# hermanjakobsen/robotic-ultrasound-imaging

Measured on AMD Instinct MI355X. Metric: env-steps/sec (whole node) at 4096 envs/GPU, random-action rollout, higher is better.
Workload: dtype f32

## Files before the change

robotic-ultrasound-imaging_amd/csrc/usim_device.h:

```cpp
#pragma once
#include <stdint.h>
#include <hip/hip_vector_types.h>

namespace usim {

constexpr int NJ = 7;
constexpr int OBS_DIM = 19;
constexpr int MAXC = 8;
constexpr int N_TOP = 99;
constexpr int LAT_NA = 9;
constexpr int LAT_NC = 11;
constexpr int LINV_BLK = 8;
constexpr int LINV_NBLK = 13;
constexpr int LOG_WIDTH = 53;
constexpr int WG = 64;

enum Field : int {
    F_Q = 0, F_QD = 7, F_Q0 = 14, F_TS = 21, F_TE = 24, F_U0 = 27, F_VBAR = 28, F_FZBAR = 29, F_FZPREV = 30,
    F_DFZ = 31, F_KST = 32, F_KDMP = 33, F_MU = 34, F_T = 35, F_TOUCH = 36, F_EPISODE = 37, F_EPRET = 38,
    F_STATUS = 39, F_NSCALAR = 40,
    F_LAT = 40,
    F_TOTAL_TOP = 40 + 200
};
__host__ __device__ inline size_t scalar_index(int f, size_t i) { return i * F_NSCALAR + f; }
// ... 36 lines not shown

struct DevModel {
    float m7, c7[3], I7[6];
    float site7[3], hand7[3];
    float pcom7[3], pI7[6];
    float torso[3];
    float grot[9];
    float gquat[4];
    float ghat[4], geps;
    float base[3];
    float ikb[3];
    float invw, wfix, wten;
    float armature[NJ];
    const float* tables;
};

struct DevCfg {
    int mode, horizon, early_term, det_traj, rand_solref, rand_pos, rand_fric, torso_drop;
    int pgs_iters, ik_iters, env_offset, adim;
    uint32_t key0, key1;
    float dt, kp_fixed, damping_ratio, kp_min, kp_max, out_pos, out_ori;
    float stiffness, damping, elem_fric, probe_fric, probe_r, probe_hl;
    float probe_hw, probe_tip;
    float probe_cull2;
    float probe_deep0, probe_inv_band;
    float probe_r2, probe_h, probe_ca, probe_cb, probe_cah;
    float top_off, y_range, drop;
    float probe_fric2, rn_scale;
    int probe_geoms;
    int pair;
    int substeps;
    float dt_ctrl;
    float frictionloss;
};

struct DevIO {
    const float* act;
    float* obs; float* rew; uint8_t* done;
    float* term_obs; int* contacts; float* ep_ret; int* ep_len;
    float* act_out;
    int* status_out;
    float* log;
    const uint8_t* mask;
    const float* reset_params;
    int2* items;
    int* count;
    int bank_row0;
    unsigned long long* dbg;
    int refill;
    int nsub;
    int block;
};

__host__ __device__ inline void advance_rollout_block(DevIO& io, size_t rows, int adim) {
    io.obs += rows * OBS_DIM; io.rew += rows; io.done += rows;
    if (io.term_obs) io.term_obs += rows * OBS_DIM;
    if (io.contacts) io.contacts += rows * (1 + MAXC);
    if (io.ep_ret) io.ep_ret += rows;
    if (io.ep_len) io.ep_len += rows;
    if (io.act_out) io.act_out += rows * adim;
}

enum LaunchFlags : int { LF_AUTO_RESET = 1, LF_RANDOM_ACT = 4 };

enum BankField : int { BQ0 = 0, BTS = 7, BTE = 10, BU0 = 13, BKST = 14, BKDMP = 15, BMU = 16, BFZ = 17, BOBS = 18, BSTATUS = 37, BANK_WORDS = 38 };
constexpr int BANK_DEPTH = 256;
// ... 9 lines not shown
```

robotic-ultrasound-imaging_amd/csrc/usim_kernels.hip:

```cpp
#include <hip/hip_runtime.h>
#include <stdint.h>
#include <type_traits>
#include "usim_device.h"
#include "usim_devmath.h"

namespace usim {


constexpr int GE_X = 0;
constexpr int GE_S = 100;
constexpr int GE_SD = 200;
constexpr int GE_A = 300;
constexpr int GE_U = 300;
constexpr int GE_U_WORDS = 144;
constexpr int CG_WORDS = 8;
constexpr int GE_CG = 400;
constexpr int GE_WS = 464;
constexpr int MAXCAND = 16;
constexpr int GE_STRIDE = 548;
static_assert(GE_WS + MAXC * 8 <= GE_STRIDE && GE_CG + (MAXCAND + 1) * CG_WORDS <= GE_STRIDE && GE_U + GE_U_WORDS <= GE_STRIDE, "per-environment LDS block overflow");
static_assert((LAT_NA + 2) * (LAT_NC + 2) <= GE_U_WORDS && LAT_NA * LAT_NC == N_TOP, "padded lattice grid");

constexpr int SOFT16_LDS_WORDS = TB_WORDS + 16 * GE_STRIDE;

// ... 89 lines not shown
    gx = bx * rn; gy = by * rn;
    const float gxi = gx * ipx;
    g = mk(copysignf(gxi * e, p.x), pxok ? copysignf(gxi * el, p.y) : gx, -gy);
    return d;
}

template <int G>
DI void collide_elem(const float* lds, float* recs, const bool valid, const int e, const int gl, const int gbase, const DevModel& M, const DevCfg& C, const float se, const float dz,
                     const f3 Kx, const f3 Ksx, const f3 Ksy, const f3 Ksz, int& nc) {
    const f3 ax = mk(lds[TB_AXIS + 3 * e], lds[TB_AXIS + 3 * e + 1], lds[TB_AXIS + 3 * e + 2]);
    const f3 tip = mk(M.torso[0] + lds[TB_POS + 3 * e], M.torso[1] + lds[TB_POS + 3 * e + 1], M.torso[2] + lds[TB_POS + 3 * e + 2] + dz) + ax * (se - ELEM_R);
    const f3 rel = tip - Kx;
    const f3 p0 = mk(dot(Ksx, rel), dot(Ksy, rel), dot(Ksz, rel));
    const f3 us = mk(dot(Ksx, ax), dot(Ksy, ax), dot(Ksz, ax)) * (-2.f * ELEM_HL);
    f3 g0, g1, gs;
    (void)probe_sdf(C, p0, g0);
    (void)probe_sdf(C, p0 + us, g1);
    const float s0 = dot(g0, us), s1 = dot(g1, us);
    const float tt = clampf(-s0 * rcp_(fmaxf(s1 - s0, 0.f) + SHAFT_EPS), 0.f, 1.f);
    const float dist = probe_sdf(C, madd(p0, us, tt), gs) - ELEM_R;
    const bool hit = valid && (dist < 0.f);
    const f3 nn = (Ksx * gs.x + Ksy * gs.y + Ksz * gs.z) * -1.f;
    const f3 rr = madd(tip, ax, -2.f * ELEM_HL * tt) + nn * (ELEM_R + 0.5f * dist) - Kx;
    const unsigned long long bal = __ballot(hit);
    const unsigned gm = (unsigned)(bal >> gbase) & ((1u << G) - 1u);
    const int slot = nc + __popc(gm & ((1u << gl) - 1u));
    const int sl = (hit && slot < MAXCAND) ? slot : MAXCAND;
    float4* rec = reinterpret_cast<float4*>(&recs[sl * CG_WORDS]);
    rec[0] = make_float4(nn.x, nn.y, nn.z, rr.x);
    rec[1] = make_float4(rr.y, rr.z, __int_as_float(e), dist);
    nc += __popc(gm);
}

DI bool collide_cull(const float* lds, const int e, const DevModel& M, const DevCfg& C, const float se, const float dz, const f3 Kx, const f3 Ksx, const f3 Ksz) {
    const f3 ax = mk(lds[TB_AXIS + 3 * e], lds[TB_AXIS + 3 * e + 1], lds[TB_AXIS + 3 * e + 2]);
    const f3 mid = mk(M.torso[0] + lds[TB_POS + 3 * e], M.torso[1] + lds[TB_POS + 3 * e + 1], M.torso[2] + lds[TB_POS + 3 * e + 2] + dz) + ax * (se - ELEM_R - ELEM_HL);
    const f3 d = mid - (Kx - Ksz * (C.probe_r + C.probe_h - C.probe_tip));
    const f3 v = d - Ksx * clampf(dot(d, Ksx), -C.probe_hl, C.probe_hl);
    return dot(v, v) < C.probe_cull2;
}
template <int G>
DI void collide_queue(const float* lds, const float* queue, const int nq, float* recs, const int gl, const int gbase, const DevModel& M, const DevCfg& C,
                      const float* s_lds, const float dz, const f3 Kx, const f3 Ksx, const f3 Ksy, const f3 Ksz, int& nc) {
    for (int j0 = 0; __any(j0 < nq); j0 += G) {
        const int j = j0 + gl;
        const bool valid = j < nq;
        const int e = valid ? __float_as_int(queue[j]) : 0;
        collide_elem<G>(lds, recs, valid, e, gl, gbase, M, C, s_lds[e], dz, Kx, Ksx, Ksy, Ksz, nc);
    }
}

#define EBF(off) lds[TB_WORDS + eb * GE_STRIDE + (off)]

template <int G>
DI void contact_overflow(float* lds, const int eb, const int gl, const int gbase, const int nc) {
    if (nc > MAXC) {
        group_sync();
        if constexpr (G == 16) {
            const int m = nc < MAXCAND ? nc : MAXCAND;
            const bool cand = gl < m;
            const float4* rec = reinterpret_cast<const float4*>(&EBF(GE_CG + gl * CG_WORDS));
            const float4 r0 = rec[0], r1 = rec[1];
            const float d = cand ? r1.w : 1.0f;
            int rank = 0;
#define USIM_RANK_STEP(I) { const float di = __int_as_float(__builtin_amdgcn_update_dpp(0, __float_as_int(d), 0x150 + I, 0xf, 0xf, true)); \
                                rank += (di < d || (di == d && I < gl)) ? 1 : 0; }
            USIM_RANK_STEP(0) USIM_RANK_STEP(1) USIM_RANK_STEP(2) USIM_RANK_STEP(3) USIM_RANK_STEP(4) USIM_RANK_STEP(5) USIM_RANK_STEP(6) USIM_RANK_STEP(7)
            USIM_RANK_STEP(8) USIM_RANK_STEP(9) USIM_RANK_STEP(10) USIM_RANK_STEP(11) USIM_RANK_STEP(12) USIM_RANK_STEP(13) USIM_RANK_STEP(14) USIM_RANK_STEP(15)
#undef USIM_RANK_STEP
            const bool keep = cand && rank < MAXC;
// ... 159 lines not shown
```

robotic-ultrasound-imaging_amd/csrc/usim_setup.h:

```cpp
#pragma once
#include <cmath>
#include <cstdint>
#include <cstring>
#include <utility>
#include <vector>

#include "../../include/usim.h"
#include "usim_device.h"
#include "usim_robot.h"

namespace usim {

enum class Mapping : int { FULL, RIGID16, SOFT16_W1, SOFT16_W2, SPLIT16, SPLIT8 };
inline bool resolve_mapping(int torso, int lanes_per_env, int waves_per_simd, int n_envs, Mapping* m) {
    if (waves_per_simd < 0 || waves_per_simd > 2) return false;
    if (torso == USIM_TORSO_NONE) { *m = Mapping::RIGID16; return lanes_per_env == 0 || lanes_per_env == 16; }
    if (lanes_per_env != 0 && lanes_per_env != 16 && lanes_per_env != 32 && lanes_per_env != 64) return false;
    const int lanes = lanes_per_env ? lanes_per_env : (waves_per_simd ? 16 : (n_envs <= 4096 ? 32 : 64));
    const int waves = waves_per_simd ? waves_per_simd : (n_envs <= 4096 ? 1 : 2);
    *m = torso == USIM_TORSO_FULL ? Mapping::FULL : lanes == 32 ? Mapping::SPLIT16 : lanes == 64 ? Mapping::SPLIT8 : (waves == 1 ? Mapping::SOFT16_W1 : Mapping::SOFT16_W2);
    return true;
}
constexpr bool soft_torso(Mapping m) { return m != Mapping::FULL && m != Mapping::RIGID16; }
constexpr bool multi_step(Mapping m) { return m != Mapping::FULL; }
constexpr int launch_steps(int remaining, int kmax, int period_left) {
    const int k = remaining < kmax ? remaining : kmax;
    return k < period_left ? k : period_left;
}
static_assert(launch_steps(1000, 256, 1) == 1, "a period with one step left");
static_assert(launch_steps(1000, 256, BANK_DEPTH) == 256 && launch_steps(1000, 64, BANK_DEPTH) == 64, "a period just refilled");
static_assert(launch_steps(1000, 1, BANK_DEPTH) == 1 && launch_steps(1000, 1, 1) == 1, "kmax = 1: one step per launch");
static_assert(launch_steps(3, 256, 200) == 3 && launch_steps(1, 256, BANK_DEPTH) == 1, "remaining smaller than everything");

// ... 203 lines not shown
    for (int id = 0; id < NSH; ++id) {
        const ShellElement& el = sh[id];
        if (el.b != 3) continue;
        const int e = el.a * 11 + el.c;
        std::memcpy(&tb[TB_SHELL + e], &id, sizeof(int));
        for (int k = 0; k < 3; ++k) { tb[TB_POS + e * 3 + k] = el.pos[k]; tb[TB_AXIS + e * 3 + k] = el.axis[k]; }
        for (int d : {0, 1, 4, 5}) if (el.nbr[d] >= 0) L[(size_t)e * N_TOP + sh[el.nbr[d]].a * 11 + sh[el.nbr[d]].c] = -kWTen;
        L[(size_t)e * N_TOP + e] = lattice_diag(el.nn);
    }
    std::vector<double> Li = invert(L, N_TOP);
    for (int i = 0; i < N_TOP; ++i) for (int j = 0; j < N_TOP; ++j) tb[TB_LINV + (size_t)i * LROW + j] = (float)Li[(size_t)i * N_TOP + j];
    return USIM_OK;
}

inline DevCfg translate_config(const usim_config& cfg) {
    DevCfg C{};
    C.mode = cfg.mode; C.horizon = cfg.horizon; C.early_term = cfg.early_termination; C.det_traj = cfg.deterministic_trajectory;
    C.rand_solref = cfg.torso_solref_randomization; C.rand_pos = cfg.initial_probe_pos_randomization; C.rand_fric = cfg.friction_randomization;
    C.torso_drop = cfg.torso_drop; C.pgs_iters = cfg.pgs_iters; C.ik_iters = cfg.ik_iters; C.env_offset = cfg.env_offset; C.adim = (cfg.mode == USIM_MODE_VARIABLE_Z) ? 7 : 6;
    C.key0 = (uint32_t)cfg.seed; C.key1 = (uint32_t)(cfg.seed >> 32);
    C.substeps = cfg.substeps > 1 ? cfg.substeps : 1;
    C.frictionloss = (float)cfg.joint_frictionloss;
    C.dt_ctrl = (float)cfg.control_dt; C.dt = (float)(cfg.control_dt / C.substeps); C.kp_fixed = (float)cfg.kp_fixed; C.damping_ratio = (float)cfg.damping_ratio; C.kp_min = (float)cfg.kp_min;
    C.kp_max = (float)cfg.kp_max; C.out_pos = (float)cfg.out_max_pos; C.out_ori = (float)cfg.out_max_ori; C.stiffness = (float)cfg.stiffness;
    C.damping = (float)cfg.damping; C.elem_fric = (float)cfg.elem_friction; C.probe_fric = (float)cfg.probe_friction;
    C.probe_geoms = cfg.probe_geoms == 2 ? 2 : 1; C.probe_fric2 = (float)cfg.probe_friction2;
    C.pair = (C.probe_geoms == 2 && cfg.pair_model != 0) ? 1 : 0; C.rn_scale = (C.probe_geoms == 2 && !C.pair) ? 0.5f : 1.0f;
    C.probe_r = (float)cfg.probe_radius; C.probe_hl = (float)cfg.probe_halflen; C.probe_hw = (float)cfg.probe_halfwidth; C.probe_tip = (float)cfg.probe_tip;
    {
        const double cb = (cfg.probe_radius - cfg.probe_radius2) / cfg.probe_height, ca = std::sqrt(1.0 - cb * cb);
        C.probe_r2 = (float)cfg.probe_radius2; C.probe_h = (float)cfg.probe_height; C.probe_ca = (float)ca; C.probe_cb = (float)cb;
        C.probe_cah = C.probe_ca * C.probe_h;
        { const double cr = cfg.probe_radius + cfg.probe_height + cfg.probe_halfwidth + 0.025 + 0.0075 + 1e-4; C.probe_cull2 = (float)(cr * cr); }
        C.probe_deep0 = (float)(cfg.probe_radius * (2.0 / 3.0)); C.probe_inv_band = (float)(1.0 / (cfg.probe_radius * (0.96 - 2.0 / 3.0)));
    }
    {
        const int shape = cfg.torso_shape ? 1 : 0;
        C.top_off = (float)kTopOff[shape]; C.y_range = (float)kYRange[shape]; C.drop = (float)(kTorsoZ[shape] - 0.0525 - 0.8);
        if (cfg.torso_drop == 0) C.drop = 0.f;
        C.torso_drop = cfg.torso_drop == 1 ? 1 : 0;
    }
    return C;
}

}
```

robotic-ultrasound-imaging_amd/csrc/usim_step16.h:

```cpp
#pragma once
#include <type_traits>

namespace usim {

template <int N, class F>
DI void static_for(F&& f) {
    if constexpr (N > 0) { static_for<N - 1>(f); f(std::integral_constant<int, N - 1>{}); }
}

template <int CTRL>
DI float dpp0(float v) { return __int_as_float(__builtin_amdgcn_update_dpp(0, __float_as_int(v), CTRL, 0xf, 0xf, true)); }
template <int G> DI int glane() { return (int)(threadIdx.x & (G - 1)); }
template <int G, int K> DI float rbc(float v) {
    if constexpr (G == 16) return dpp0<0x150 + K>(v);
    else {
        const int iv = __float_as_int(v);
        const int t = __builtin_amdgcn_update_dpp(iv, iv, 0x150 + K, 0xf, 0x3, false);
        return __int_as_float(__builtin_amdgcn_update_dpp(t, iv, 0x150 + 8 + K, 0xf, 0xc, false));
    }
}
template <int G, int D> DI float rshr0(float v) {
    const float t = dpp0<0x110 + D>(v);
    if constexpr (G == 16) return t; else return (glane<G>() < D) ? 0.f : t;
}
// ... 135 lines not shown
    arow = arow > 5 ? 5 : arow;
    const float4 j0 = *reinterpret_cast<const float4*>(&xl[arow * 8]), j1 = *reinterpret_cast<const float4*>(&xl[arow * 8 + 4]);
    Jr[0] = j0.x; Jr[1] = j0.y; Jr[2] = j0.z; Jr[3] = j0.w; Jr[4] = j1.x; Jr[5] = j1.y; Jr[6] = j1.z; Jr[7] = j1.w;
}

template <int G>
DI float solve6_task(float* A, float b, const int gl) {
    static_for<6>([&](auto Kc) {
        constexpr int k = decltype(Kc)::value;
        constexpr int lk = TASK_LANE[k];
        const float g = (A[k] - (gl == lk ? 1.f : 0.f)) * rcp_(rbc<G, lk>(A[k]));
#pragma unroll
        for (int c = k + 1; c < 6; ++c) A[c] = fmaf(-g, rbc<G, lk>(A[c]), A[c]);
        b = fmaf(-g, rbc<G, lk>(b), b);
    });
    return b;
}

constexpr int X16_WORDS = 64;
constexpr int X16_RIGID_STRIDE = 84;

#ifndef USIM_WPR16
#define USIM_WPR16 4
#endif
#ifndef USIM_WPR8
#define USIM_WPR8 4
#endif
template <int G> constexpr int wpr() { return G == 16 ? USIM_WPR16 : USIM_WPR8; }
constexpr int MB_POSE = X16_WORDS;
constexpr int MB_OP = MB_POSE + 12;
constexpr int MB_W = MB_OP + 64;
constexpr int MB_Q = MB_W + 16;
constexpr int MB_GOAL = MB_Q + 100;
constexpr int X2_STRIDE = MB_GOAL + 12;
template <int G> constexpr int x2_base() { return TB_WORDS + (64 * wpr<G>() / G) * GE_STRIDE; }
static_assert(x2_base<16>() % 4 == 0 && x2_base<8>() % 4 == 0 && X2_STRIDE % 4 == 0 && MB_OP % 4 == 0 && MB_W % 4 == 0, "mailbox block: 16-byte accesses");
static_assert((x2_base<8>() + 32 * X2_STRIDE) * 4 <= 160 * 1024, "split kernel with 8-lane groups: LDS of a CU");
template <int G> constexpr int arm_cull_rounds() { return 7; }

#if defined(USIM_TSTAMP) || defined(USIM_TSTAMP_NOWAIT)
#define USIM_BAR() do { __syncthreads(); ++nbar; } while (0)
#else
#define USIM_BAR() __syncthreads()
#endif


constexpr int ARM_LDS_WORDS = A16_LANES * AT_STRIDE;
template <int TORSO, int ROLE, int G> constexpr int arm_lds_base();
template <int NE, class WR = NoWarm>
struct Carry {
    float dqj, qdj, q0j;
    Episode ep;
    float s[NE], sd[NE];
    WR wr;
};

template <int TORSO, int ROLE, int G> constexpr int arm_lds_base() {
    return ROLE != 0 ? x2_base<G>() + (64 * wpr<G>() / G) * X2_STRIDE : (TORSO ? SOFT16_LDS_WORDS : 16 * X16_RIGID_STRIDE);
}
static_assert((arm_lds_base<1, 1, 8>() + ARM_LDS_WORDS) * 4 <= 160 * 1024 && arm_lds_base<1, 1, 8>() % 4 == 0 && arm_lds_base<1, 1, 16>() % 4 == 0 && arm_lds_base<1, 0, 16>() % 4 == 0
              && arm_lds_base<0, 0, 16>() % 4 == 0, "arm table behind the LDS blocks of every 16-lane kernel");

template <int TORSO, int MODE, int ROLE, int NT, int G = 16, bool RES = false, class WR = NoWarm>
DI void step16_one(float* lds, const DevModel& M, const DevCfg& C, float* __restrict__ st, const int n, const int npad, const DevIO& io, const int flags, const long long rstep,
                   const bool first_pass, const int sub, int& nbar, Carry<TORSO ? (N_TOP + G - 1) / G : 1, WR>& cy) {
    constexpr bool WARM = !std::is_same<WR, NoWarm>::value;
    static_assert(!WARM || (TORSO == 1 && ROLE == 0) || (TORSO == 1 && MODE == 0), "warm start: the soft-torso kernels");
    constexpr int WPR = (ROLE != 0) ? wpr<G>() : 4;
    constexpr int EPW = 64 / G, EPB = WPR * EPW;
    static_assert(!RES || MODE == 0, "resident state: step launches only");
    constexpr int X2_BASE = x2_base<G>();
    constexpr unsigned GMASK = (G == 16) ? 0xffffu : 0xffu;
    static_assert(G == 16 || (TORSO == 1 && MODE == 0 && ROLE != 0), "8-lane groups: the split soft-torso step only");
    constexpr int NE = TORSO ? (N_TOP + G - 1) / G : 1;
    static_assert(ROLE == 0 || (TORSO == 1 && MODE == 0), "the split kernel is the soft-torso step");
    const int lane = threadIdx.x & 63, wave = (threadIdx.x >> 6) & (WPR - 1);
    constexpr bool RES_HERE = RES && !(ROLE == 2 && G == 16);
    const bool fresh = !RES_HERE || first_pass;
    const int gl = lane & (G - 1), ge = lane / G;
    const int gbase = lane - gl;
    const int eb = wave * EPW + ge;
    const bool auto_reset = (flags & LF_AUTO_RESET) != 0;
    unsigned long long* const dbg = io.dbg;
    const bool refill = (MODE == 1) && io.refill != 0;
    const int item_cnt = refill ? io.count[0] : 1;
    const int item_first = refill ? (int)blockIdx.x * EPB : 0;
    for (int item0 = item_first; item0 < item_cnt; item0 += refill ? (int)gridDim.x * EPB : 1) {
    int env = blockIdx.x * EPB + eb;
    bool valid = env < n;
    int item_ep = 0;
    if (refill) {
        valid = item0 + eb < item_cnt;
        const int2 it = valid ? io.items[item0 + eb] : make_int2(0, 0);
        env = it.x; item_ep = it.y;
    }
    const bool store = valid && gl == 0;
    const int ei = valid ? env : (refill ? 0 : n - 1);
#define LAT(w) st[(size_t)F_LAT * npad + (size_t)ei * LAT_ENV_WORDS + (w)]
// ... 94 lines not shown
    const bool last_sub = sub == C.substeps - 1;
    const int tphys = (MODE == 0) ? (t - 1) * C.substeps + sub : 0;
    const float dt = C.dt, inv_h = rcp_((float)C.horizon);
#if defined(USIM_TSTAMP) || defined(USIM_TSTAMP_NOWAIT)
#define RSTAMP(k) do { if (dbg && blockIdx.x == 0 && (threadIdx.x & (64 * WPR - 1)) == 0) dbg[(ROLE == 2 ? 30 : 20) + (k)] = __builtin_readcyclecounter(); } while (0)
#else
#define RSTAMP(k) do { } while (0)
#endif
#define XSTAMP(k) RSTAMP(20 + (k))
    if constexpr (ROLE == 2) {
        RSTAMP(0);
        float* const mb = &lds[mbo];
        const int* tb_shell = reinterpret_cast<const int*>(lds + TB_SHELL);
        float dz, vz, az;
        torso_motion(C, tphys, dz, vz, az);
        lattice_rhs<G, NE>(lds, eb, gl, M, az, kst, kdmp, true, s_pre, sd_pre);
        lattice_solve<G>(lds, eb, gl, gbase);
        RSTAMP(1);
        USIM_BAR();
        RSTAMP(2);
        const f3 xs = mk(mb[MB_POSE], mb[MB_POSE + 1], mb[MB_POSE + 2]), sy = mk(mb[MB_POSE + 3], mb[MB_POSE + 4], mb[MB_POSE + 5]),
                 sz = mk(mb[MB_POSE + 6], mb[MB_POSE + 7], mb[MB_POSE + 8]);
        const f3 sxc = cross(sy, sz);
        int nq = __float_as_int(mb[MB_POSE + 10]);
#pragma unroll
        for (int i = arm_cull_rounds<G>(); i < NE; ++i) {
            const int eraw = i * G + gl, e = eraw < N_TOP ? eraw : N_TOP - 1;
            const bool cand = (eraw < N_TOP) && collide_cull(lds, e, M, C, s_pre[i], dz, xs, sxc, sz);
            const unsigned gm = (unsigned)(__ballot(cand) >> gbase) & GMASK;
            mb[MB_Q + (cand ? nq + __popc(gm & ((1u << gl) - 1u)) : 99)] = __int_as_float(e);
            nq += __popc(gm);
        }
        group_sync();
        int nc = 0;
        collide_queue<G>(lds, mb + MB_Q, nq, &EB(GE_CG), gl, gbase, M, C, &EB(GE_S), dz, xs, sxc, sy, sz, nc);
        constexpr bool EARLY = G == 8;
        ContactRows P;
        int nc_early = nc, overflow_early = 0, ncmax_early = 0, cel_early[MAXC];
        if constexpr (EARLY) {
            contact_overflow<G>(lds, eb, gl, gbase, nc_early);
            if (nc_early > MAXC) { overflow_early = 1; nc_early = MAXC; }
            group_sync();
#pragma unroll
            for (int k = MAXC; k >= 1; --k) if (ncmax_early == 0 && __any(nc_early >= k)) ncmax_early = k;
#pragma unroll
            for (int k = 0; k < MAXC; ++k) cel_early[k] = (k < nc_early) ? __float_as_int(EB(GE_CG + k * CG_WORDS + 6)) : 0;
            if (ncmax_early > 0) contact_rows<G>(lds, eb, gl, M, C, nc_early, cel_early, vz, P);
        }
        RSTAMP(3);
        USIM_BAR();
        RSTAMP(4);
        if constexpr (!EARLY) contact_overflow<G>(lds, eb, gl, gbase, nc);
        int overflow = 0;
        if (nc > MAXC) { overflow = 1; nc = MAXC; }
        if constexpr (!EARLY) group_sync();
        XSTAMP(0);
        int ncmax = 0;
        if constexpr (EARLY) { nc = nc_early; overflow = overflow_early; ncmax = ncmax_early; }
        else {
#pragma unroll
            for (int k = MAXC; k >= 1; --k) if (ncmax == 0 && __any(nc >= k)) ncmax = k;
        }
        XSTAMP(1);
        float gf[MAXC], W[6] = {0, 0, 0, 0, 0, 0};
        int cel[MAXC];
#pragma unroll
        for (int k = 0; k < MAXC; ++k) { const int ek = __float_as_int(EB(GE_CG + k * CG_WORDS + 6)); gf[k] = 0.f; cel[k] = EARLY ? cel_early[k] : ((k < nc) ? ek : 0); }
        if (ncmax > 0) {
            float alpha[6], vs[6], Lp[21];
#pragma unroll
            for (int a = 0; a < 6; ++a) {
                alpha[a] = mb[MB_OP + 48 + a]; vs[a] = mb[MB_OP + 54 + a];
#pragma unroll
                for (int b = 0; b <= a; ++b) Lp[PK(a, b)] = mb[MB_OP + a * 8 + b];
            }
            XSTAMP(2);
            contact_solve<G, EARLY, true>(lds, eb, gl, M, C, nc, ncmax, cel, Lp, alpha, vs, mu, vz, P, W, gf, dbg, cy.wr);
            XSTAMP(3);
        } else warm_clear(cy.wr);
        if (gl == 0) {
            *reinterpret_cast<float4*>(&mb[MB_W]) = make_float4(W[0], W[1], W[2], W[3]);
            *reinterpret_cast<float4*>(&mb[MB_W + 4]) = make_float4(W[4], W[5], __int_as_float(nc), __int_as_float(overflow));
#pragma unroll
            for (int k = 0; k < MAXC; ++k) { const int sh = tb_shell[cel[k]]; mb[MB_W + 8 + k] = __int_as_float((k < nc) ? sh : -1); }
        }
        RSTAMP(5);
        USIM_BAR();
        RSTAMP(6);
        {
            float acc_e[NE];
#pragma unroll
            for (int i = 0; i < NE; ++i) { const int e = gl + i * G; acc_e[i] = (e < N_TOP) ? EB(GE_A + e) : 0.f; }
#pragma unroll
            for (int k = 0; k < MAXC; ++k) {
#pragma unroll
                for (int i = 0; i < NE; ++i) {
                    const int e = (gl + i * G < N_TOP) ? gl + i * G : N_TOP - 1;
                    acc_e[i] = fmaf(lds[TB_LINV + e * LROW + cel[k]], gf[k], acc_e[i]);
                }
            }
// ... 96 lines not shown
    fk16<G>(at, qj, X, Y, Z, P);
    const f3 rcm = X * at[AT_LCOM] + Y * at[AT_LCOM + 1] + Z * at[AT_LCOM + 2];
    const f3 cm_ = P + rcm;
    const f3 sx = rbc3<G, 7>(X), sy = rbc3<G, 7>(Y), sz = rbc3<G, 7>(Z), xs = rbc3<G, 7>(P);
    const f3 hand = rbc3<G, NJ - 1>(P + X * M.hand7[0] + Y * M.hand7[1] + Z * M.hand7[2]);
    if constexpr (ROLE == 1) {
        {
            float dz_, vz_, az_;
            torso_motion(C, tphys, dz_, vz_, az_);
            const f3 sxc = cross(sy, sz);
            int nq = 0;
#pragma unroll
            for (int i = 0; i < NE; ++i) {
                const int eraw = i * G + gl, e = eraw < N_TOP ? eraw : N_TOP - 1;
                if (eraw < N_TOP) EB(GE_S + eraw) = s_pre[i];
                if (i >= arm_cull_rounds<G>()) continue;
                const bool cand = (eraw < N_TOP) && collide_cull(lds, e, M, C, s_pre[i], dz_, xs, sxc, sz);
                const unsigned gm = (unsigned)(__ballot(cand) >> gbase) & GMASK;
                xl[MB_Q + (cand ? nq + __popc(gm & ((1u << gl) - 1u)) : 99)] = __int_as_float(e);
                nq += __popc(gm);
            }
            if (gl == 0) xl[MB_POSE + 10] = __int_as_float(nq);
        }
        if (gl == 7) {
            float* mbp = xl + MB_POSE;
            mbp[0] = P.x; mbp[1] = P.y; mbp[2] = P.z; mbp[3] = Y.x; mbp[4] = Y.y; mbp[5] = Y.z; mbp[6] = Z.x; mbp[7] = Z.y; mbp[8] = Z.z;
        }
        if constexpr (ROLE == 1) RSTAMP(1);
        USIM_BAR();
        if constexpr (ROLE == 1) RSTAMP(2);
    }

    float act[7] = {0, 0, 0, 0, 0, 0, 0};
    if constexpr (MODE == 0) {
    if constexpr (ROLE != 2) {
    if (flags & LF_RANDOM_ACT) {
        const uint32_t gid = (uint32_t)(C.env_offset + ei);
        const u4 r = philox(gid, (uint32_t)rstep, (uint32_t)((unsigned long long)rstep >> 32), 1u + (uint32_t)(gl & 1), C.key0, C.key1);
        const float ra = __uint_as_float(r.a), rb = __uint_as_float(r.b), rc = __uint_as_float(r.c), rd = __uint_as_float(r.d);
        uint32_t rr[7];
        rr[0] = __float_as_uint(rbc<G, 0>(ra)); rr[1] = __float_as_uint(rbc<G, 0>(rb)); rr[2] = __float_as_uint(rbc<G, 0>(rc)); rr[3] = __float_as_uint(rbc<G, 0>(rd));
        rr[4] = __float_as_uint(rbc<G, 1>(ra)); rr[5] = __float_as_uint(rbc<G, 1>(rb)); rr[6] = __float_as_uint(rbc<G, 1>(rc));
#pragma unroll
        for (int a = 0; a < 7; ++a) {
            const float u = u01(rr[a]);
            const bool sgn = (C.mode == 1) || (C.mode == 3) || (C.mode == 2 && a == 6);
            act[a] = sgn ? 2.f * u - 1.f : u;
            if (C.mode == 3) act[a] *= WRENCH_MAX;
        }
        if (io.act_out && store) {
#pragma unroll
            for (int a = 0; a < 7; ++a) if (a < C.adim) io.act_out[(size_t)ei * C.adim + a] = act[a];
        }
    } else {
#pragma unroll
        for (int a = 0; a < 7; ++a) if (a < C.adim) act[a] = finite_or_zero(io.act[(size_t)ei * C.adim + a]);
    }
    }
    }
    float bias, Mr[NJ];
    f3 w, al, ao;
    {
        const f3 zq = Z * qdj;
        w = prefix_sum<G>(zq);
        const f3 wp = w - zq;
        const f3 dal = cross(wp, zq);
        al = prefix_sum<G>(dal);
        const f3 alp = al - dal;
        const f3 r = mk(P.x - rshr0<G, 1>(P.x), P.y - rshr0<G, 1>(P.y), P.z - rshr0<G, 1>(P.z));
        f3 da = cross(alp, r) + cross(wp, cross(wp, r));
        da.z += (gl == 0) ? GRAV : 0.f;
        ao = prefix_sum<G>(da);
        const f3 ac = ao + cross(al, rcm) + cross(w, cross(w, rcm));
        const float mass = at[AT_MASS];
        const f3 F = ac * mass;
        const float* I = &at[AT_INERTIA];
        const f3 RI0 = mk(X.x * I[0] + Y.x * I[1] + Z.x * I[2], X.x * I[1] + Y.x * I[3] + Z.x * I[4], X.x * I[2] + Y.x * I[4] + Z.x * I[5]);
        const f3 RI1 = mk(X.y * I[0] + Y.y * I[1] + Z.y * I[2], X.y * I[1] + Y.y * I[3] + Z.y * I[4], X.y * I[2] + Y.y * I[4] + Z.y * I[5]);
        const f3 RI2 = mk(X.z * I[0] + Y.z * I[1] + Z.z * I[2], X.z * I[1] + Y.z * I[3] + Z.z * I[4], X.z * I[2] + Y.z * I[4] + Z.z * I[5]);
        float Iw[6];
        Iw[0] = RI0.x * X.x + RI0.y * Y.x + RI0.z * Z.x; Iw[1] = RI0.x * X.y + RI0.y * Y.y + RI0.z * Z.y; Iw[2] = RI0.x * X.z + RI0.y * Y.z + RI0.z * Z.z;
        Iw[3] = RI1.x * X.y + RI1.y * Y.y + RI1.z * Z.y; Iw[4] = RI1.x * X.z + RI1.y * Y.z + RI1.z * Z.z; Iw[5] = RI2.x * X.z + RI2.y * Y.z + RI2.z * Z.z;
        const f3 Nc = symmul(Iw, al) + cross(w, symmul(Iw, w)) + cross(cm_, F);
        const f3 fa = suffix_sum<G>(F), na = suffix_sum<G>(Nc);
        bias = dot(Z, na - cross(P, fa));
// ... 163 lines not shown
        difference_quat(qe, M.gquat, obs + 15);
        if constexpr (MODE == 0) {
            float pe0 = 90.f * (xw.x - tpw.x), pe1 = 90.f * (xw.y - tpw.y);
            pe0 *= pe0; pe1 *= pe1;
            pos_err_norm = sqrt_(pe0 * pe0 + pe1 * pe1);
            pos_rew = 5.f * exp_(-pos_err_norm);
            const float qc[4] = {qe[3], qe[0], qe[1], qe[2]};
            ori_err = 0.2f * distance_quat_goal(qc, M.ghat, M.geps);
            ori_rew = exp_(-ori_err);
            float ve = 45.f * (vbar - 0.04f); ve *= ve;
            vel_rew = exp_(-ve);
            float fe = 0.7f * (fzbar - 5.f); fe *= fe;
            force_e = 3.f * exp_(-fe);
            float de = 0.01f * dfz; de *= de;
            dforce_e = 2.f * exp_(-de);
        }
    };
    float W[6] = {0, 0, 0, 0, 0, 0};
    int ncon = 0, overflow = 0, con_shell[MAXC];
#pragma unroll
    for (int k = 0; k < MAXC; ++k) con_shell[k] = -1;
    if constexpr (ROLE == 1) {
        if (is_task) {
            const int arow = blk ? 3 + comp : comp;
            float* mbo = xl + MB_OP;
            *reinterpret_cast<float4*>(&mbo[arow * 8]) = make_float4(Li[0], Li[1], Li[2], Li[3]);
            mbo[arow * 8 + 4] = Li[4]; mbo[arow * 8 + 5] = Li[5];
            mbo[48 + arow] = alpha_t; mbo[54 + arow] = v6;
        }
        RSTAMP(3);
        USIM_BAR();
        RSTAMP(4);
        precompute();
        RSTAMP(5);
        USIM_BAR();
        RSTAMP(6);
        const float4 w0 = *reinterpret_cast<const float4*>(&xl[MB_W]), w1 = *reinterpret_cast<const float4*>(&xl[MB_W + 4]);
        W[0] = w0.x; W[1] = w0.y; W[2] = w0.z; W[3] = w0.w; W[4] = w1.x; W[5] = w1.y;
        ncon = __float_as_int(w1.z); overflow = __float_as_int(w1.w);
#pragma unroll
        for (int k = 0; k < MAXC; ++k) con_shell[k] = __float_as_int(xl[MB_W + 8 + k]);
    } else if constexpr (TORSO != 0) {
        const int* tb_shell = reinterpret_cast<const int*>(lds + TB_SHELL);
        float dz, vz, az;
        torso_motion(C, tphys, dz, vz, az);
        lattice_rhs<G, NE>(lds, eb, gl, M, az, kst, kdmp, MODE == 0, s_pre, sd_pre);
        USIM_STAMP(dbg, 5);
        int nc = collide_all<G, NE>(lds, eb, gl, gbase, M, C, MODE == 0, s_pre, dz, xs, sy, sz);
        lattice_solve<G>(lds, eb, gl, gbase);
        contact_overflow<G>(lds, eb, gl, gbase, nc);
        USIM_STAMP(dbg, 7);
        if (nc > MAXC) { overflow = 1; nc = MAXC; }
        ncon = nc;
        group_sync();
        int ncmax = 0;
#pragma unroll
        for (int k = MAXC; k >= 1; --k) if (ncmax == 0 && __any(nc >= k)) ncmax = k;
        float gf[MAXC];
        int cel[MAXC];
#pragma unroll
        for (int k = 0; k < MAXC; ++k) { gf[k] = 0.f; cel[k] = (k < nc) ? __float_as_int(EB(GE_CG + k * CG_WORDS + 6)) : 0; }
        if (ncmax > 0) {
            float alpha[6], vs[6], Lp[21];
            static_for<6>([&](auto Ac) {
                constexpr int a = decltype(Ac)::value;
                alpha[a] = rbc<G, TASK_LANE[a]>(alpha_t); vs[a] = rbc<G, TASK_LANE[a]>(v6);
// ... 205 lines not shown
        }
        if (gl == 0) {
            float4* s4 = reinterpret_cast<float4*>(so);
            if (need) {
                so[F_TS] = ts.x; so[F_TS + 1] = ts.y; so[F_TS + 2] = ts.z;
                s4[6] = make_float4(te.x, te.y, te.z, u0);
            }
            s4[7] = make_float4(vbar, fzbar, fzprev, dfz);
            s4[8] = make_float4(kst, kdmp, mu, __int_as_float(t));
            s4[9] = make_float4(__int_as_float(touched), __int_as_float(episode), epret, __int_as_float(status));
        }
    }
    if (refill) group_sync();
    }
    if (MODE == 1 && refill) work_list_close(io);
    USIM_STAMP(dbg, 16);
    if constexpr (ROLE == 1) RSTAMP(9);
#undef RSTAMP
#undef XSTAMP
#undef LAT
#undef EB
}

template <int TORSO, int MODE, int ROLE, int NT, bool MULTI = false, int G = 16, class WR = NoWarm, bool ACTS = false>
DI void step16_body(float* lds, const DevModel& M, const DevCfg& C, float* __restrict__ st, const int n, const int npad, const DevIO& io0, const int flags, const long long rstep) {
    const int S = (MULTI && MODE == 0 && C.substeps > 1) ? C.substeps : 1;
    const int nsub = (MULTI && MODE == 0) ? (io0.nsub > 1 ? io0.nsub : 1) * S : 1;
    DevIO io = io0;
    int nbar = 0;
    Carry<TORSO ? (N_TOP + G - 1) / G : 1, WR> cy;
    int sub = 0;
    long long cstep = rstep;
    for (int ks = 0; ks < nsub; ++ks) {
        step16_one<TORSO, MODE, ROLE, NT, G, MULTI && MODE == 0, WR>(lds, M, C, st, n, npad, io, flags, cstep, ks == 0, sub, nbar, cy);
        const bool ctrl_done = sub == S - 1;
        if (ctrl_done) { sub = 0; ++cstep; } else ++sub;
        if (ks + 1 < nsub) {
            __threadfence_block();
            if constexpr (ROLE != 0) USIM_BAR();
            if (io0.block && ctrl_done) advance_rollout_block(io, (size_t)n, C.adim);
            if constexpr (ACTS) { if (ctrl_done) io.act += (size_t)n * C.adim; }
        }
    }
#if defined(USIM_TSTAMP) || defined(USIM_TSTAMP_NOWAIT)
    if (ROLE != 0 && io0.dbg && blockIdx.x == 0 && (threadIdx.x & (64 * wpr<G>() - 1)) == 0) io0.dbg[ROLE == 1 ? 46 : 47] = (unsigned long long)nbar;
#endif
}

template <int TORSO, int OCC, int MODE, bool MULTI = false, bool WARM = false>
__global__ __launch_bounds__(256) __attribute__((amdgpu_waves_per_eu(OCC, OCC))) void usim_step16_kernel(const DevModel M, const DevCfg C, float* __restrict__ st, int n, int npad,
                                                                                                          const DevIO io, int flags, long long rstep) {
    extern __shared__ __attribute__((aligned(16))) float lds[];
    step16_body<TORSO, MODE, 0, 256, MULTI, 16, typename std::conditional<WARM, WarmOf<16>::type, NoWarm>::type>(lds, M, C, st, n, npad, io, flags, rstep);
}

template <int TORSO, int OCC, bool WARM = false>
__global__ __launch_bounds__(256) __attribute__((amdgpu_waves_per_eu(OCC, OCC))) void usim_step16_acts_kernel(const DevModel M, const DevCfg C, float* __restrict__ st, int n, int npad,
                                                                                                               const DevIO io, int flags, long long rstep) {
    extern __shared__ __attribute__((aligned(16))) float lds[];
    step16_body<TORSO, 0, 0, 256, true, 16, typename std::conditional<WARM, WarmOf<16>::type, NoWarm>::type, true>(lds, M, C, st, n, npad, io, flags, rstep);
}

template <bool MULTI, int G = 16, bool WARM = false>
__global__ __launch_bounds__(128 * wpr<G>()) __attribute__((amdgpu_waves_per_eu(2, 2))) void usim_step32_kernel(const DevModel* __restrict__ Mp, const DevCfg* __restrict__ Cp, float* __restrict__ st, int n, int npad,
                                                                                                                  const DevIO io, int flags, long long rstep) {
    extern __shared__ __attribute__((aligned(16))) float lds[];
    const DevModel& M = *Mp; const DevCfg& C = *Cp;
// ... 19 lines not shown
```

Baseline: 231.8 million.

## Tighten probe cull to element capsule, draw next random action ahead during precompute

Replaces the probe-axis cull test with a capsule test along each element axis, using a new host-computed radius, so fewer shell elements enter the collision queue. In the resident split kernel the arm wave draws the next step's random action while it waits through the precompute barrier and parks it in a mailbox slot, taking the philox draw off the critical path. It also adds an optional early contact-list path with a readlane max over the 16-lane groups, and sets the 16-lane arm cull rounds to zero by default. The tighter cull changes which candidates are kept, so correctness depends on the new bound being conservative.

```diff
diff --git a/robotic-ultrasound-imaging_amd/csrc/usim_device.h b/robotic-ultrasound-imaging_amd/csrc/usim_device.h
--- a/robotic-ultrasound-imaging_amd/csrc/usim_device.h
+++ b/robotic-ultrasound-imaging_amd/csrc/usim_device.h
@@ -92,6 +92,7 @@
     int substeps;
     float dt_ctrl;
     float frictionloss;
+    float probe_cull2c;
 };
 
 struct DevIO {
diff --git a/robotic-ultrasound-imaging_amd/csrc/usim_kernels.hip b/robotic-ultrasound-imaging_amd/csrc/usim_kernels.hip
--- a/robotic-ultrasound-imaging_amd/csrc/usim_kernels.hip
+++ b/robotic-ultrasound-imaging_amd/csrc/usim_kernels.hip
@@ -145,10 +145,18 @@
     nc += __popc(gm);
 }
 
+#ifndef USIM_CULL_CAPSULE
+#define USIM_CULL_CAPSULE 1
+#endif
+constexpr bool CULL_CAPSULE = USIM_CULL_CAPSULE != 0;
 DI bool collide_cull(const float* lds, const int e, const DevModel& M, const DevCfg& C, const float se, const float dz, const f3 Kx, const f3 Ksx, const f3 Ksz) {
     const f3 ax = mk(lds[TB_AXIS + 3 * e], lds[TB_AXIS + 3 * e + 1], lds[TB_AXIS + 3 * e + 2]);
     const f3 mid = mk(M.torso[0] + lds[TB_POS + 3 * e], M.torso[1] + lds[TB_POS + 3 * e + 1], M.torso[2] + lds[TB_POS + 3 * e + 2] + dz) + ax * (se - ELEM_R - ELEM_HL);
     const f3 d = mid - (Kx - Ksz * (C.probe_r + C.probe_h - C.probe_tip));
+    if constexpr (CULL_CAPSULE) {
+        const f3 v = d - ax * clampf(dot(d, ax), -ELEM_HL, ELEM_HL);
+        return dot(v, v) < C.probe_cull2c;
+    }
     const f3 v = d - Ksx * clampf(dot(d, Ksx), -C.probe_hl, C.probe_hl);
     return dot(v, v) < C.probe_cull2;
 }
diff --git a/robotic-ultrasound-imaging_amd/csrc/usim_setup.h b/robotic-ultrasound-imaging_amd/csrc/usim_setup.h
--- a/robotic-ultrasound-imaging_amd/csrc/usim_setup.h
+++ b/robotic-ultrasound-imaging_amd/csrc/usim_setup.h
@@ -1,4 +1,5 @@
 #pragma once
+#include <algorithm>
 #include <cmath>
 #include <cstdint>
 #include <cstring>
@@ -268,6 +269,11 @@
         C.probe_r2 = (float)cfg.probe_radius2; C.probe_h = (float)cfg.probe_height; C.probe_ca = (float)ca; C.probe_cb = (float)cb;
         C.probe_cah = C.probe_ca * C.probe_h;
         { const double cr = cfg.probe_radius + cfg.probe_height + cfg.probe_halfwidth + 0.025 + 0.0075 + 1e-4; C.probe_cull2 = (float)(cr * cr); }
+        {
+            const double hh = std::hypot(cfg.probe_halflen, cfg.probe_halfwidth);
+            const double rp = std::max(std::hypot(hh, cfg.probe_height) + cfg.probe_radius, hh + cfg.probe_radius2), cr = rp + 0.0075 + 1e-4;
+            C.probe_cull2c = (float)(cr * cr);
+        }
         C.probe_deep0 = (float)(cfg.probe_radius * (2.0 / 3.0)); C.probe_inv_band = (float)(1.0 / (cfg.probe_radius * (0.96 - 2.0 / 3.0)));
     }
     {
diff --git a/robotic-ultrasound-imaging_amd/csrc/usim_step16.h b/robotic-ultrasound-imaging_amd/csrc/usim_step16.h
--- a/robotic-ultrasound-imaging_amd/csrc/usim_step16.h
+++ b/robotic-ultrasound-imaging_amd/csrc/usim_step16.h
@@ -191,11 +191,23 @@
 constexpr int MB_W = MB_OP + 64;
 constexpr int MB_Q = MB_W + 16;
 constexpr int MB_GOAL = MB_Q + 100;
-constexpr int X2_STRIDE = MB_GOAL + 12;
+#ifndef USIM_DRAW_AHEAD
+#define USIM_DRAW_AHEAD 1
+#endif
+constexpr bool DRAW_AHEAD = USIM_DRAW_AHEAD != 0;
+#ifndef USIM_LIST_AHEAD
+#define USIM_LIST_AHEAD 0
+#endif
+constexpr bool LIST_AHEAD = USIM_LIST_AHEAD != 0;
+constexpr int MB_ACT = MB_GOAL + 12;
+constexpr int X2_STRIDE = MB_ACT + (DRAW_AHEAD ? 8 : 0);
 template <int G> constexpr int x2_base() { return TB_WORDS + (64 * wpr<G>() / G) * GE_STRIDE; }
-static_assert(x2_base<16>() % 4 == 0 && x2_base<8>() % 4 == 0 && X2_STRIDE % 4 == 0 && MB_OP % 4 == 0 && MB_W % 4 == 0, "mailbox block: 16-byte accesses");
+static_assert(x2_base<16>() % 4 == 0 && x2_base<8>() % 4 == 0 && X2_STRIDE % 4 == 0 && MB_OP % 4 == 0 && MB_W % 4 == 0 && MB_ACT % 4 == 0, "mailbox block: 16-byte accesses");
 static_assert((x2_base<8>() + 32 * X2_STRIDE) * 4 <= 160 * 1024, "split kernel with 8-lane groups: LDS of a CU");
-template <int G> constexpr int arm_cull_rounds() { return 7; }
+#ifndef USIM_ARM_CULL16
+#define USIM_ARM_CULL16 0
+#endif
+template <int G> constexpr int arm_cull_rounds() { return G == 16 ? USIM_ARM_CULL16 : 7; }
 
 #if defined(USIM_TSTAMP) || defined(USIM_TSTAMP_NOWAIT)
 #define USIM_BAR() do { __syncthreads(); ++nbar; } while (0)
@@ -220,9 +232,10 @@
 static_assert((arm_lds_base<1, 1, 8>() + ARM_LDS_WORDS) * 4 <= 160 * 1024 && arm_lds_base<1, 1, 8>() % 4 == 0 && arm_lds_base<1, 1, 16>() % 4 == 0 && arm_lds_base<1, 0, 16>() % 4 == 0
               && arm_lds_base<0, 0, 16>() % 4 == 0, "arm table behind the LDS blocks of every 16-lane kernel");
 
-template <int TORSO, int MODE, int ROLE, int NT, int G = 16, bool RES = false, class WR = NoWarm>
+template <int TORSO, int MODE, int ROLE, int NT, int G = 16, bool RES = false, class WR = NoWarm, bool AHEAD = false>
 DI void step16_one(float* lds, const DevModel& M, const DevCfg& C, float* __restrict__ st, const int n, const int npad, const DevIO& io, const int flags, const long long rstep,
-                   const bool first_pass, const int sub, int& nbar, Carry<TORSO ? (N_TOP + G - 1) / G : 1, WR>& cy) {
+                   const bool first_pass, const int sub, const bool more, int& nbar, Carry<TORSO ? (N_TOP + G - 1) / G : 1, WR>& cy) {
+    static_assert(!AHEAD || (ROLE == 1 && RES), "action drawn ahead: the arm wave of a resident split launch");
     constexpr bool WARM = !std::is_same<WR, NoWarm>::value;
     static_assert(!WARM || (TORSO == 1 && ROLE == 0) || (TORSO == 1 && MODE == 0), "warm start: the soft-torso kernels");
     constexpr int WPR = (ROLE != 0) ? wpr<G>() : 4;
@@ -383,31 +396,41 @@
             nq += __popc(gm);
         }
         group_sync();
+#if defined(USIM_TSTAMP) || defined(USIM_TSTAMP_NOWAIT)
+        if (dbg && blockIdx.x == 0 && wave == 0 && gl == 0) dbg[54 + ge] = 1ull + (unsigned long long)nq;
+#endif
         int nc = 0;
         collide_queue<G>(lds, mb + MB_Q, nq, &EB(GE_CG), gl, gbase, M, C, &EB(GE_S), dz, xs, sxc, sy, sz, nc);
         constexpr bool EARLY = G == 8;
         ContactRows P;
+        constexpr bool LIST_EARLY = EARLY || (G == 16 && LIST_AHEAD);
         int nc_early = nc, overflow_early = 0, ncmax_early = 0, cel_early[MAXC];
-        if constexpr (EARLY) {
+        if constexpr (LIST_EARLY) {
             contact_overflow<G>(lds, eb, gl, gbase, nc_early);
             if (nc_early > MAXC) { overflow_early = 1; nc_early = MAXC; }
             group_sync();
-#pragma unroll
-            for (int k = MAXC; k >= 1; --k) if (ncmax_early == 0 && __any(nc_early >= k)) ncmax_early = k;
+            if constexpr (G == 16) {
+                const int m01 = max(__builtin_amdgcn_readlane(nc_early, 0), __builtin_amdgcn_readlane(nc_early, 16));
+                const int m23 = max(__builtin_amdgcn_readlane(nc_early, 32), __builtin_amdgcn_readlane(nc_early, 48));
+                ncmax_early = max(m01, m23);
+            } else {
+#pragma unroll
+                for (int k = MAXC; k >= 1; --k) if (ncmax_early == 0 && __any(nc_early >= k)) ncmax_early = k;
+            }
 #pragma unroll
             for (int k = 0; k < MAXC; ++k) cel_early[k] = (k < nc_early) ? __float_as_int(EB(GE_CG + k * CG_WORDS + 6)) : 0;
-            if (ncmax_early > 0) contact_rows<G>(lds, eb, gl, M, C, nc_early, cel_early, vz, P);
+            if constexpr (EARLY) { if (ncmax_early > 0) contact_rows<G>(lds, eb, gl, M, C, nc_early, cel_early, vz, P); }
         }
         RSTAMP(3);
         USIM_BAR();
         RSTAMP(4);
-        if constexpr (!EARLY) contact_overflow<G>(lds, eb, gl, gbase, nc);
+        if constexpr (!LIST_EARLY) contact_overflow<G>(lds, eb, gl, gbase, nc);
         int overflow = 0;
         if (nc > MAXC) { overflow = 1; nc = MAXC; }
-        if constexpr (!EARLY) group_sync();
+        if constexpr (!LIST_EARLY) group_sync();
         XSTAMP(0);
         int ncmax = 0;
-        if constexpr (EARLY) { nc = nc_early; overflow = overflow_early; ncmax = ncmax_early; }
+        if constexpr (LIST_EARLY) { nc = nc_early; overflow = overflow_early; ncmax = ncmax_early; }
         else {
 #pragma unroll
             for (int k = MAXC; k >= 1; --k) if (ncmax == 0 && __any(nc >= k)) ncmax = k;
@@ -416,7 +439,7 @@
         float gf[MAXC], W[6] = {0, 0, 0, 0, 0, 0};
         int cel[MAXC];
 #pragma unroll
-        for (int k = 0; k < MAXC; ++k) { const int ek = __float_as_int(EB(GE_CG + k * CG_WORDS + 6)); gf[k] = 0.f; cel[k] = EARLY ? cel_early[k] : ((k < nc) ? ek : 0); }
+        for (int k = 0; k < MAXC; ++k) { const int ek = __float_as_int(EB(GE_CG + k * CG_WORDS + 6)); gf[k] = 0.f; cel[k] = LIST_EARLY ? cel_early[k] : ((k < nc) ? ek : 0); }
         if (ncmax > 0) {
             float alpha[6], vs[6], Lp[21];
 #pragma unroll
@@ -579,11 +602,9 @@
     }
 
     float act[7] = {0, 0, 0, 0, 0, 0, 0};
-    if constexpr (MODE == 0) {
-    if constexpr (ROLE != 2) {
-    if (flags & LF_RANDOM_ACT) {
+    auto draw_action = [&](const long long cs, float (&a7)[7]) {
         const uint32_t gid = (uint32_t)(C.env_offset + ei);
-        const u4 r = philox(gid, (uint32_t)rstep, (uint32_t)((unsigned long long)rstep >> 32), 1u + (uint32_t)(gl & 1), C.key0, C.key1);
+        const u4 r = philox(gid, (uint32_t)cs, (uint32_t)((unsigned long long)cs >> 32), 1u + (uint32_t)(gl & 1), C.key0, C.key1);
         const float ra = __uint_as_float(r.a), rb = __uint_as_float(r.b), rc = __uint_as_float(r.c), rd = __uint_as_float(r.d);
         uint32_t rr[7];
         rr[0] = __float_as_uint(rbc<G, 0>(ra)); rr[1] = __float_as_uint(rbc<G, 0>(rb)); rr[2] = __float_as_uint(rbc<G, 0>(rc)); rr[3] = __float_as_uint(rbc<G, 0>(rd));
@@ -592,12 +613,36 @@
         for (int a = 0; a < 7; ++a) {
             const float u = u01(rr[a]);
             const bool sgn = (C.mode == 1) || (C.mode == 3) || (C.mode == 2 && a == 6);
-            act[a] = sgn ? 2.f * u - 1.f : u;
-            if (C.mode == 3) act[a] *= WRENCH_MAX;
+            a7[a] = sgn ? 2.f * u - 1.f : u;
+            if (C.mode == 3) a7[a] *= WRENCH_MAX;
+        }
+    };
+    auto keep_action = [&](const float (&a7)[7]) {
+        if (gl == 0) {
+            *reinterpret_cast<float4*>(&xl[MB_ACT]) = make_float4(a7[0], a7[1], a7[2], a7[3]);
+            *reinterpret_cast<float4*>(&xl[MB_ACT + 4]) = make_float4(a7[4], a7[5], a7[6], 0.f);
+        }
+    };
+    if constexpr (MODE == 0) {
+    if constexpr (ROLE != 2) {
+    if (flags & LF_RANDOM_ACT) {
+        if (AHEAD && !first_pass) {
+            const float4 a0 = *reinterpret_cast<const float4*>(&xl[MB_ACT]), a1 = *reinterpret_cast<const float4*>(&xl[MB_ACT + 4]);
+            act[0] = a0.x; act[1] = a0.y; act[2] = a0.z; act[3] = a0.w; act[4] = a1.x; act[5] = a1.y; act[6] = a1.z;
+        } else {
+            draw_action(rstep, act);
+            if constexpr (AHEAD) keep_action(act);
         }
         if (io.act_out && store) {
-#pragma unroll
-            for (int a = 0; a < 7; ++a) if (a < C.adim) io.act_out[(size_t)ei * C.adim + a] = act[a];
+            if constexpr (AHEAD) {
+                float* const ao = io.act_out + (size_t)ei * C.adim;
+#pragma unroll
+                for (int a = 0; a < 6; ++a) ao[a] = act[a];
+                if (C.adim > 6) ao[6] = act[6];
+            } else {
+#pragma unroll
+                for (int a = 0; a < 7; ++a) if (a < C.adim) io.act_out[(size_t)ei * C.adim + a] = act[a];
+            }
         }
     } else {
 #pragma unroll
@@ -827,6 +872,13 @@
         USIM_BAR();
         RSTAMP(4);
         precompute();
+        if constexpr (AHEAD) {
+            if ((flags & LF_RANDOM_ACT) && more && last_sub) {
+                float nxt[7];
+                draw_action(rstep + 1, nxt);
+                keep_action(nxt);
+            }
+        }
         RSTAMP(5);
         USIM_BAR();
         RSTAMP(6);
@@ -1098,7 +1150,8 @@
     int sub = 0;
     long long cstep = rstep;
     for (int ks = 0; ks < nsub; ++ks) {
-        step16_one<TORSO, MODE, ROLE, NT, G, MULTI && MODE == 0, WR>(lds, M, C, st, n, npad, io, flags, cstep, ks == 0, sub, nbar, cy);
+        constexpr bool AHEAD = DRAW_AHEAD && ROLE == 1 && MULTI && MODE == 0 && !ACTS;
+        step16_one<TORSO, MODE, ROLE, NT, G, MULTI && MODE == 0, WR, AHEAD>(lds, M, C, st, n, npad, io, flags, cstep, ks == 0, sub, ks + 1 < nsub, nbar, cy);
         const bool ctrl_done = sub == S - 1;
         if (ctrl_done) { sub = 0; ++cstep; } else ++sub;
         if (ks + 1 < nsub) {
```

Result: faster. 236.7 million (median of 6 runs) (+2.1%).
